# mumianyuxin/M3DSSD

Hardware: AMD Instinct MI355X
Metric: images/sec at 1280x384 bs=8, 1/2/4/8 MI355X; 3D-box Linf vs ref (higher is better)
Workload: dtype f32; 1 GPU; BASELINE.json configs[1]: full M3d_inference_align (DLA-34 + DCNv2 align + ANAB) forward + decode + top-3000 + NMS, bs=8/GPU, 1280x384, fp32, random-init synthetic weights and frames; per_gpu_batch=8, global_batch=8, parallelism=dp1 (batch sharded, 1 all-gather of [B,40,14] detections)

## Files before the change

### include/m3dssd_hip.h

```cpp
#ifndef M3DSSD_HIP_H
#define M3DSSD_HIP_H

#include <stdint.h>

#ifdef __cplusplus
extern "C" {
#endif

typedef void *m3d_stream_t;

enum {
    M3D_OK = 0,
    M3D_E_ARG = -1,
    M3D_E_HIP = -2,
    M3D_E_WORKSPACE = -3
};

const char *m3d_last_error(void);
#define M3D_ABI_VERSION 5
int m3d_abi_version(void);
const char *m3d_source_hashes(void);

typedef struct m3d_conv_desc {
    const float *in;
// ... 17 lines not shown
    int sigmoid_from;
    const float *dcn_offmask;
    int dcn_om_cs;
    float *splitk_ws;
    long long splitk_ws_bytes;
} m3d_conv_desc;

int m3d_conv2d_forward(const m3d_conv_desc *d, m3d_stream_t stream);
int m3d_conv2d_splitk_plan(const m3d_conv_desc *d, int *splits, long long *ws_bytes);

int m3d_conv_wave_applicable(const m3d_conv_desc *d);
int m3d_conv_wave_splitk_plan(const m3d_conv_desc *d, int *splits, long long *ws_bytes);
int m3d_conv_wave_forward(const m3d_conv_desc *d, m3d_stream_t stream);
int m3d_conv_wave_forward_wgsplit(const m3d_conv_desc *d, m3d_stream_t stream);
int m3d_conv_wave_wgsplit_width(const m3d_conv_desc *d, int *slices, int *width);

int m3d_wino_conv3x3_forward(const m3d_conv_desc *d, m3d_stream_t stream);
int m3d_wino_conv3x3_variant(const m3d_conv_desc *d);
int m3d_wino_conv3x3_splitk_plan(const m3d_conv_desc *d, int *splits, long long *ws_bytes);
int m3d_wino_conv3x3_forward_ex(const m3d_conv_desc *d, int variant, m3d_stream_t stream);
int m3d_wino44_applicable(const m3d_conv_desc *d);
int m3d_wino44_conv3x3_forward(const m3d_conv_desc *d, m3d_stream_t stream);
int m3d_wino44_conv3x3_forward_ex(const m3d_conv_desc *d, int nb, m3d_stream_t stream);
int m3d_wino44_kpair(const m3d_conv_desc *d);
int m3d_wino44_splitk_plan(const m3d_conv_desc *d, int *splits, long long *ws_bytes);
int m3d_wino44_conv3x3_forward_touch(const m3d_conv_desc *d, int nb, const void *touch, long long touch_bytes, m3d_stream_t stream);

int m3d_cache_touch(const void *p, long long bytes, m3d_stream_t stream);
int m3d_upload_indirect(const void *const *src_slot, void *dst, long long bytes, m3d_stream_t stream);

// ... 315 lines not shown
```

### m3dssd_amd/_hip.py

```python
import ctypes
import os
import subprocess

_HERE = os.path.dirname(os.path.abspath(__file__))
CSRC = os.path.join(_HERE, "csrc")
SO_PATH = os.environ.get("M3D_HIP_LIB") or os.path.join(CSRC, "build", "libm3dssd_hip.so")
HEADER = os.path.join(os.path.dirname(_HERE), "include", "m3dssd_hip.h")

c_int, c_float, c_ll, c_void_p = ctypes.c_int, ctypes.c_float, ctypes.c_longlong, ctypes.c_void_p


class ConvDesc(ctypes.Structure):
    _fields_ = [
        ("inp", c_void_p), ("in_cs", c_int),
        ("N", c_int), ("H", c_int), ("W", c_int), ("Cin", c_int),
        ("wgt", c_void_p), ("wgt_img_stride", c_ll),
        ("Cout", c_int), ("Cout_pad", c_int),
        ("kh", c_int), ("kw", c_int), ("stride", c_int), ("pad", c_int), ("dil", c_int),
        ("Ho", c_int), ("Wo", c_int),
        ("out", c_void_p), ("out_cs", c_int), ("out_nchw", c_int), ("out_img_stride", c_ll),
        ("scale", c_void_p), ("shift", c_void_p),
        ("res", c_void_p), ("res_cs", c_int), ("res_mode", c_int),
        ("act", c_int), ("sigmoid_from", c_int),
        ("dcn_offmask", c_void_p), ("dcn_om_cs", c_int),
# ... 113 lines not shown
    "m3d_wino_conv3x3_splitk_plan": (c_int, [ctypes.POINTER(ConvDesc), ctypes.POINTER(c_int), ctypes.POINTER(c_ll)]),
    "m3d_wino_conv3x3_variant": (c_int, [ctypes.POINTER(ConvDesc)]),
    "m3d_wino44_applicable": (c_int, [ctypes.POINTER(ConvDesc)]),
    "m3d_wino44_conv3x3_forward": (c_int, [ctypes.POINTER(ConvDesc), P]),
    "m3d_wino44_conv3x3_forward_ex": (c_int, [ctypes.POINTER(ConvDesc), c_int, P]),
    "m3d_wino44_kpair": (c_int, [ctypes.POINTER(ConvDesc)]),
    "m3d_wino44_conv3x3_forward_touch": (c_int, [ctypes.POINTER(ConvDesc), c_int, P, c_ll, P]),
    "m3d_cache_touch": (c_int, [P, c_ll, P]),
    "m3d_upload_indirect": (c_int, [P, P, c_ll, P]),
    "m3d_wino44_splitk_plan": (c_int, [ctypes.POINTER(ConvDesc), ctypes.POINTER(c_int), ctypes.POINTER(c_ll)]),
    "m3d_conv_wave_applicable": (c_int, [ctypes.POINTER(ConvDesc)]),
    "m3d_conv_wave_splitk_plan": (c_int, [ctypes.POINTER(ConvDesc), ctypes.POINTER(c_int), ctypes.POINTER(c_ll)]),
    "m3d_conv_wave_forward": (c_int, [ctypes.POINTER(ConvDesc), P]),
    "m3d_conv_wave_forward_wgsplit": (c_int, [ctypes.POINTER(ConvDesc), P]),
    "m3d_conv_wave_wgsplit_width": (c_int, [ctypes.POINTER(ConvDesc), ctypes.POINTER(c_int), ctypes.POINTER(c_int)]),
    "m3d_conv2d_tile": (c_int, [ctypes.POINTER(ConvDesc)] + [ctypes.POINTER(c_int)] * 4),
    "m3d_conv2d_splitk_plan": (c_int, [ctypes.POINTER(ConvDesc), ctypes.POINTER(c_int), ctypes.POINTER(c_ll)]),
    "m3d_dcn_v2_workspace_bytes": (c_ll, [c_int] * 10),
    "m3d_dcn_v2_workspace_bytes_grouped": (c_ll, [c_int] * 11),
    "m3d_dcn_v2_forward": (c_int, [P] * 6 + [c_int] * 14 + [P, c_ll, P]),
    "m3d_dcn_v2_backward_workspace_bytes": (c_ll, [c_int] * 11),
    "m3d_dcn_v2_backward": (c_int, [P] * 10 + [c_int] * 14 + [P, c_ll, P]),
    "m3d_rpn_loss_workspace_bytes": (c_ll, [c_int, c_ll]),
    "m3d_rpn_targets": (c_int, [P, c_int, c_int, c_int, P, c_int, P, c_int, c_int, P, P, c_int, P, P, P, P, P, c_ll, P]),
    "m3d_rpn_loss": (c_int, [P, c_int, c_int, c_int, P, c_int, P, c_int, c_int, P, P, P, c_int, P, P, P, P, P, P, P, P, P, P, c_ll, P]),
    "m3d_pack_conv_weight": (c_int, [P, P] + [c_int] * 6 + [P]),
    "m3d_nchw_to_nhwc": (c_int, [P, P] + [c_int] * 5 + [P]),
    "m3d_nhwc_to_nchw": (c_int, [P, c_int, P] + [c_int] * 4 + [P]),
    "m3d_stem_conv7x7": (c_int, [P, P, P, P, P] + [c_int] * 4 + [P]),
    "m3d_refine_3d": (c_int, [P, P, c_int, c_int, P, P, ctypes.c_double, c_int, ctypes.c_double, ctypes.c_double, P, P]),
# ... 92 lines not shown
```

### m3dssd_amd/csrc/dcn_wave.hip

```cpp
#include <stdlib.h>

#include <type_traits>

#include "common.h"

struct ConvWaveArgs {
    const float *in, *wfrag, *scale, *shift, *res, *om;
    float *out;
    int in_cs, out_cs, res_cs, om_cs;
    int H, W, Cin, Ho, Wo, HoWo, Cout;
    int kh, kw, stride, pad, dil;
    int M, KG, tiles_n;
    int act, res_mode, sigmoid_from;
    int vec_out;
    long long w_img_stride;
    unsigned in_bytes, out_bytes, res_bytes, w_bytes;
    float *ws;
    int splits, ss_per, base_waves;
    unsigned ws_bytes;
#ifdef CONV_TRACE
    long long *trace;
#endif
};


#ifdef CONV_TRACE
static long long *g_conv_trace = nullptr;
extern "C" void m3d_conv_wave_set_trace(void *buf) { g_conv_trace = (long long *)buf; }
static int g_conv_variant = 0;
extern "C" void m3d_conv_wave_set_variant(int v) { g_conv_variant = v; }
#define TRACE_INIT() long long *trp = (a.trace && threadIdx.x < 64) ? a.trace + (size_t)blockIdx.x * 128 : nullptr; int tri = 0
#define TRACE() do { if (trp && lane == 0 && tri < 128) trp[tri++] = __builtin_readcyclecounter(); } while (0)
#else
#define TRACE_INIT()
#define TRACE()
#endif

template <bool DEFORM, int NT, int NCQ = 4, int WPE = (DEFORM ? 2 : 3), int S = 1>
__global__ __launch_bounds__(64 * S) __attribute__((amdgpu_waves_per_eu(WPE))) void conv_wave_kernel(const ConvWaveArgs a)
{
    __shared__ __attribute__((aligned(16))) float tileS[S * 32 * 32];
    __shared__ __attribute__((aligned(16))) float tapst[(DEFORM ? 9 : 1) * 32 * 8];
    const int lane = threadIdx.x & 63, l31 = lane & 31, h = lane >> 5;
    const int wv = S > 1 ? __builtin_amdgcn_readfirstlane((int)threadIdx.x >> 6) : 0;
    float *const tileA = tileS + wv * 1024;
    const int gp = lane >> 3, gc = lane & 7;
    TRACE_INIT();
    TRACE();
    int blk;
    {
        const int nblk = gridDim.x, bid = blockIdx.x;
        const int q = nblk >> 3, r = nblk & 7, xcd = bid & 7, loc = bid >> 3;
        blk = (xcd < r ? xcd * (q + 1) : r * (q + 1) + (xcd - r) * q) + loc;
    }
    int split = wv;
    if (S == 1 && a.splits > 1) {
        split = blk / a.base_waves;
        blk -= split * a.base_waves;
    }
    const int bm = blk / a.tiles_n, bn = blk - bm * a.tiles_n;
    const int m0 = bm * 32;
    const int KK = a.kh * a.kw, C32 = a.Cin / 32;
    const bool idle = S > 1 && wv >= a.splits;
    const int ss0 = idle ? 0 : split * a.ss_per, ss1 = idle ? 0 : min(KK * C32, ss0 + a.ss_per);

    const __amdgpu_buffer_rsrc_t rin = make_rsrc(a.in, a.in_bytes);
// ... 111 lines not shown
    };

    f32x16 acc[NT];
#pragma unroll
    for (int nt = 0; nt < NT; ++nt)
#pragma unroll
        for (int r = 0; r < 16; ++r) acc[nt][r] = 0.f;

    int tap, c32;
    constexpr bool cmaj = DEFORM;
    if constexpr (cmaj) { c32 = ss0 / KK; tap = ss0 - c32 * KK; }
    else { tap = ss0 / C32; c32 = ss0 - tap * C32; }
    setup_tap(tap);
    issue_gather(c32);
    issue_b((tap * C32 + c32) * 4, bfA);

    unsigned wr_off[4], rd_off[4];
#pragma unroll
    for (int g = 0; g < 4; ++g) {
        const int r = 8 * g + gp;
        wr_off[g] = (unsigned)(r * 32 + ((gc ^ ((r >> 1) & 7)) * 4));
    }
#pragma unroll
    for (int j = 0; j < 4; ++j) rd_off[j] = (unsigned)(l31 * 32 + (((2 * j + h) ^ ((l31 >> 1) & 7)) * 4));

    TRACE();
    for (int st = ss0; st < ss1; ++st) {
        TRACE();
        const int kg0 = (tap * C32 + c32) * 4;
#pragma unroll
// ... 229 lines not shown
                const int m = mb + (r & 3) + 8 * (r >> 2);
                const unsigned ro = (cok && m < a.M) ? ((unsigned)m * (unsigned)a.res_cs + (unsigned)co) * 4u : M3D_BUF_OOB;
                rv[r] = __builtin_bit_cast(float, __builtin_amdgcn_raw_buffer_load_b32(rres, ro, 0, 0));
            }
        }
#pragma unroll
        for (int r = 0; r < 16; ++r) {
            const int m = mb + (r & 3) + 8 * (r >> 2);
            float v = conv_epi_affine(acc[nt][r], sc, sh, a.res ? rv[r] : 0.f, a.res != nullptr, a.res_mode);
            v = conv_epi_act(v, a.sigmoid_from >= 0 && co >= a.sigmoid_from, a.act == 1 ? M3D_LEAKY_SLOPE : 1.f);
            const unsigned oo = (cok && m < a.M) ? ((unsigned)m * (unsigned)a.out_cs + (unsigned)co) * 4u : M3D_BUF_OOB;
            __builtin_amdgcn_raw_buffer_store_b32(__builtin_bit_cast(unsigned, v), rout, oo, 0, 0);
        }
    }
    TRACE();
}

static int conv_wave_plan(const m3d_conv_desc *d, bool enforce_min, int *splits, int *ss_per, bool allow32 = false)
{
    *splits = 1;
    *ss_per = d->kh * d->kw * (d->Cin / 32);
    if (d->out_nchw) return 0;
    if (d->dcn_offmask && d->kh * d->kw > 9) return 0;
    if (d->Cin % 32 != 0 || d->Cout_pad % 32 != 0) return 0;
    if (d->Cout_pad % 64 != 0 && (!allow32 || d->dcn_offmask || d->wgt_img_stride)) return 0;
    const int cw = d->Cout_pad % 128 == 0 ? 128 : (d->Cout_pad % 64 == 0 ? 64 : 32);
    if (d->wgt_img_stride && (d->Ho * d->Wo) % 32 != 0) return 0;
    const long long M = (long long)d->N * d->Ho * d->Wo;
    const long long base = ((M + 31) / 32) * (d->Cout_pad / cw);
    if (base >= (1ll << 28)) return 0;
// ... 34 lines not shown
    *ws_bytes = (*splits > 1 && d->Cout_pad % 64 == 0) ? (long long)*splits * d->N * d->Ho * d->Wo * d->Cout_pad * 4 : 0;
    return M3D_OK;
}

template <bool DEFORM, int NT>
static void launch_wgsplit(const ConvWaveArgs &a, int S, int wgs, hipStream_t stream)
{
    constexpr int WPE = DEFORM ? 2 : 3;
    switch (S) {
    case 2: hipLaunchKernelGGL((conv_wave_kernel<DEFORM, NT, 4, WPE, 2>), dim3(wgs), dim3(128), 0, stream, a); break;
    case 4: hipLaunchKernelGGL((conv_wave_kernel<DEFORM, NT, 4, WPE, 4>), dim3(wgs), dim3(256), 0, stream, a); break;
    default: hipLaunchKernelGGL((conv_wave_kernel<DEFORM, NT, 4, WPE, 8>), dim3(wgs), dim3(512), 0, stream, a); break;
    }
}

static int conv_wave_run(const m3d_conv_desc *d_, hipStream_t stream, bool wgsplit)
{
    M3D_REQUIRE(d_ && d_->in && d_->wgt && d_->out, "conv_wave: null pointer");
    m3d_conv_desc dd = *d_;
    static float dummy;
    if (wgsplit) { dd.splitk_ws = &dummy; dd.splitk_ws_bytes = 0; }
    const m3d_conv_desc *d = &dd;
    int splits = 1, ss_per = 0;
    const int waves = conv_wave_plan(d, false, &splits, &ss_per, wgsplit);
    M3D_REQUIRE(waves > 0, "conv_wave: needs Cin %% 32 == 0, Cout_pad %% 64 == 0 (%% 32: plain, shared weights, wgsplit entry), NHWC output, "
                           "Ho*Wo %% 32 == 0 with per-image weights");
    const int ho = (d->H + 2 * d->pad - (d->dil * (d->kh - 1) + 1)) / d->stride + 1;
    const int wo = (d->W + 2 * d->pad - (d->dil * (d->kw - 1) + 1)) / d->stride + 1;
    M3D_REQUIRE(ho == d->Ho && wo == d->Wo, "conv_wave: Ho/Wo mismatch");
    M3D_REQUIRE(d->in_cs % 32 == 0 && d->in_cs >= d->Cin && ((uintptr_t)d->in & 127) == 0 && ((uintptr_t)d->wgt & 15) == 0,
                "conv_wave: the input view must be 128-byte aligned with in_cs %% 32 == 0");
    const long long M = (long long)d->N * d->Ho * d->Wo;
    M3D_REQUIRE(!d->wgt_img_stride || (d->wgt_img_stride % 4 == 0 && d->stride == 1 && d->Ho == d->H && d->Wo == d->W),
                "conv_wave: per-image weights need an image-aligned 16-byte stride and a same-size output");
    M3D_REQUIRE((long long)d->N * d->H * d->W * d->in_cs * 4 < (1ll << 31) && M * d->out_cs * 4 < (1ll << 31) &&
                M * d->res_cs * 4 < (1ll << 31) && (long long)d->Cout_pad * d->kh * d->kw * d->Cin * 4 < (1ll << 31),
                "conv_wave: views must be < 2 GiB");
    ConvWaveArgs a;
    a.in = d->in; a.wfrag = d->wgt; a.scale = d->scale; a.shift = d->shift; a.res = d->res; a.om = d->dcn_offmask;
    a.out = d->out;
    a.in_cs = d->in_cs; a.out_cs = d->out_cs; a.res_cs = d->res_cs; a.om_cs = d->dcn_om_cs;
    a.H = d->H; a.W = d->W; a.Cin = d->Cin; a.Ho = d->Ho; a.Wo = d->Wo; a.HoWo = d->Ho * d->Wo; a.Cout = d->Cout;
    a.kh = d->kh; a.kw = d->kw; a.stride = d->stride; a.pad = d->pad; a.dil = d->dil;
    const int cw = d->Cout_pad % 128 == 0 ? 128 : (d->Cout_pad % 64 == 0 ? 64 : 32);
    a.M = (int)M; a.KG = d->kh * d->kw * d->Cin / 8; a.tiles_n = d->Cout_pad / cw;
    a.act = d->act; a.res_mode = d->res_mode; a.sigmoid_from = d->sigmoid_from; a.w_img_stride = d->wgt_img_stride;
    static int vec_epi = -1;
    if (vec_epi < 0) { const char *e = getenv("M3D_WAVE_VEC_EPILOGUE"); vec_epi = e ? atoi(e) : 1; }
    a.vec_out = vec_epi && d->out_cs % 4 == 0 && ((uintptr_t)d->out & 15) == 0 &&
                (!d->res || (d->res_cs % 4 == 0 && ((uintptr_t)d->res & 15) == 0)) &&
                (!d->scale || ((uintptr_t)d->scale & 15) == 0) && (!d->shift || ((uintptr_t)d->shift & 15) == 0);
    a.in_bytes = (unsigned)((long long)d->N * d->H * d->W * d->in_cs * 4);
    a.out_bytes = (unsigned)(M * d->out_cs * 4);
    a.res_bytes = (unsigned)(M * d->res_cs * 4);
    a.w_bytes = (unsigned)((long long)cw * d->kh * d->kw * d->Cin * 4);
#ifdef CONV_TRACE
    a.trace = g_conv_trace;
#endif
    a.ws = nullptr; a.splits = 1; a.ss_per = ss_per; a.base_waves = waves; a.ws_bytes = 0;
    if (splits > 1 && wgsplit) {
        const int S = splits <= 2 ? 2 : (splits <= 4 ? 4 : 8);
        M3D_REQUIRE(splits <= 8, "conv_wave: %d K slices do not fit a workgroup", splits);
        a.splits = splits; a.base_waves = waves / splits;
        if (cw == 128) {
            if (d->dcn_offmask) launch_wgsplit<true, 4>(a, S, a.base_waves, stream);
            else launch_wgsplit<false, 4>(a, S, a.base_waves, stream);
        } else if (cw == 64) {
            if (d->dcn_offmask) launch_wgsplit<true, 2>(a, S, a.base_waves, stream);
            else launch_wgsplit<false, 2>(a, S, a.base_waves, stream);
        } else {
            launch_wgsplit<false, 1>(a, S, a.base_waves, stream);
        }
        M3D_LAUNCH_CHECK();
        return M3D_OK;
// ... 31 lines not shown
    if (splits > 1) {
        SplitkReduceArgs r;
        r.ws = a.ws; r.scale = d->scale; r.shift = d->shift; r.res = d->res; r.out = d->out;
        r.M = (int)M; r.Cout = d->Cout; r.Cout_pad = d->Cout_pad; r.splits = splits; r.out_cs = d->out_cs; r.res_cs = d->res_cs;
        r.res_mode = d->res_mode; r.act = d->act; r.sigmoid_from = d->sigmoid_from;
        return m3d_launch_splitk_reduce(r, stream);
    }
    return M3D_OK;
}

extern "C" int m3d_conv_wave_forward(const m3d_conv_desc *d, m3d_stream_t stream)
{
    return conv_wave_run(d, (hipStream_t)stream, false);
}

extern "C" int m3d_conv_wave_wgsplit_width(const m3d_conv_desc *d, int *slices, int *width)
{
    M3D_REQUIRE(d && slices && width, "conv_wave_wgsplit_width: null pointer");
    m3d_conv_desc t = *d;
    static float dummy;
    t.splitk_ws = &dummy;
    int p;
    const int waves = conv_wave_plan(&t, false, slices, &p, true);
    M3D_REQUIRE(waves > 0 && *slices <= 8, "conv_wave_wgsplit_width: the wave kernel does not apply to this descriptor");
    *width = *slices <= 1 ? 1 : (*slices <= 2 ? 2 : (*slices <= 4 ? 4 : 8));
    return M3D_OK;
}

extern "C" int m3d_conv_wave_forward_wgsplit(const m3d_conv_desc *d, m3d_stream_t stream)
{
// ... 3 lines not shown
```

### m3dssd_amd/engine.py

```python
import ctypes
import math
import os

import numpy as np
import torch

from . import _hip
from ._hip import ConvDesc, MlpDesc
from .config import model_flags

BN_EPS = 1e-5
SELECT_KEYS = os.environ.get("M3D_SELECT_KEYS", "1") != "0"
PSP_SIZES = (1, 4, 8, 16)
BACKBONE_CHANNELS = {"dla34": (16, 32, 64, 128, 256, 512), "dla102": (16, 32, 128, 256, 512, 1024)}
DLA102_LEVELS = (1, 1, 1, 3, 4, 1)


def _rup(a, b):
    return (a + b - 1) // b * b


class View:
    __slots__ = ("t", "ptr", "n", "h", "w", "c", "cs", "keep")

# ... 103 lines not shown
def pack_wino44_c16(weight, device):
    g = weight.detach().to("cpu", torch.float64)
    assert tuple(g.shape) == (16, 16, 3, 3)
    u = torch.einsum("ai,ocij,bj->abco", _WINO44_G, g, _WINO44_G).reshape(36, 4, 4, 16)
    return u.permute(0, 1, 3, 2).contiguous().to(torch.float32).reshape(-1).to(device)


WINO_MIN_BLOCKS = int(os.environ.get("M3D_WINO_MIN_BLOCKS", "128"))
FUSED_ANAB = os.environ.get("M3D_FUSED_ANAB", "1") != "0"
USE_ANAB_WAVE = os.environ.get("M3D_ANAB_WAVE", "1") != "0"
USE_ANAB_NESTED = os.environ.get("M3D_ANAB_NESTED", "1") != "0"
USE_DCN_WAVE = os.environ.get("M3D_DCN_WAVE", "1") != "0"
USE_CONV_WAVE = os.environ.get("M3D_CONV_WAVE", "1") != "0"
USE_CONV_WAVE_WGSPLIT = os.environ.get("M3D_CONV_WAVE_WGSPLIT", "1") != "0"
USE_OFFMASK_WAVE = os.environ.get("M3D_OFFMASK_WAVE", "1") != "0"
USE_WINO = os.environ.get("M3D_WINO", "1") != "0"
USE_WINO44 = os.environ.get("M3D_WINO44", "1") != "0"
WINO44_TOUCH = os.environ.get("M3D_WINO44_TOUCH", "1") != "0"
WINO44_TOUCH_SPAN = int(os.environ.get("M3D_WINO44_TOUCH_SPAN", "2"))
USE_WINO44_SPLITK = os.environ.get("M3D_WINO44_SPLITK", "1") != "0"
W44_SPLIT_NB = 2 if os.environ.get("M3D_W44_SPLIT_NB", "1") == "2" else 1
W44_SPLIT_KPAIR = os.environ.get("M3D_W44_SPLIT_NB", "1") == "3"
WINO44_MIN_WGS = int(os.environ.get("M3D_WINO44_MIN_WGS", "1000000"))
WINO44_MIN_WGS_NB1 = int(os.environ.get("M3D_WINO44_MIN_WGS_NB1", "200"))


class OpCost:

    def __init__(self, hbm_bytes):
        self.hbm_bytes = int(hbm_bytes)


def lo_hi_contains(start, end, n, br):
    lo, hi = start, (n if end is None else end)
    return lo <= br[0] and br[2] <= hi


class _Plan:

    def __init__(self):
        self.ops = []
        self.keep = []
        self.named = {}
        self.w44_prev = None
        self.branches = []


class Engine:
    def __init__(self, state_dict, conf, device=None, backbone_only=False):
        self.L = _hip.lib()
        self.backbone_only = backbone_only
        self.device = torch.device(device if device is not None else conf.device)
        if self.device.type != "cuda":
            raise NotImplementedError("the M3DSSD HIP engine runs on a ROCm device only (got %s)" % self.device)
        if self.device.index is None:
            self.device = torch.device("cuda", torch.cuda.current_device())
        self.conf = conf
        self.back_bone = str(conf.back_bone) if "back_bone" in conf else "dla34"
        if self.back_bone not in BACKBONE_CHANNELS:
            raise NotImplementedError("back_bone %r: the engine runs %s" % (self.back_bone, " / ".join(BACKBONE_CHANNELS)))
# ... 201 lines not shown
            if ssplits.value > 1:
                ws = torch.empty(sbytes.value // 4, device=self.device, dtype=torch.float32)
                plan.keep.append(ws)
                d.splitk_ws, d.splitk_ws_bytes = ws.data_ptr(), sbytes.value
                nb, ks44 = W44_SPLIT_NB, ssplits.value
        if w44ok and nb:
            u44 = pc.wino44()
            plan.keep.append(u44)
            d.wgt = u44.data_ptr()
            flops = 2.0 * x.n * d.Ho * d.Wo * d.Cout * 9 * pc.cin
            nxt = {"ptr": None, "bytes": 0}
            if WINO44_TOUCH:
                nbytes = u44.numel() * 4
                if plan.w44_prev is not None and len(plan.ops) - plan.w44_prev[0] <= WINO44_TOUCH_SPAN:
                    plan.w44_prev[1]["ptr"], plan.w44_prev[1]["bytes"] = u44.data_ptr(), nbytes
                else:
                    plan.ops.append((name + ".touch", "touch", 0.0,
                                     lambda st: _hip.check(L.m3d_cache_touch(u44.data_ptr(), nbytes, st)), OpCost(nbytes)))
            plan.w44_prev = (len(plan.ops), nxt)
            kp = ",kpair" if (nb == 1 and ((ks44 == 1 and L.m3d_wino44_kpair(ref) == 1) or (ks44 > 1 and W44_SPLIT_KPAIR))) else ""
            plan.ops.append((name, "wino44<16,%d%s%s>" % (16 * nb, ",splitk%d" % ks44 if ks44 > 1 else "", kp), flops,
                             lambda st: _hip.check(L.m3d_wino44_conv3x3_forward_touch(ref, nb, nxt["ptr"], nxt["bytes"], st)), d))
            return
        if (pc is not None and wgt_ptr is None and getattr(pc, "wino", None) is not None and kh == 3 and kw == 3
                and stride == 1 and pad == 1 and om is None and planar is None and x.h % 2 == 0 and x.w % 2 == 0
                and wino_blocks >= WINO_MIN_BLOCKS):
            d.wgt = pc.wino.data_ptr()
            flops = 2.0 * x.n * d.Ho * d.Wo * d.Cout * 9 * pc.cin
            ssplits, sbytes = ctypes.c_int(), ctypes.c_longlong()
            _hip.check(L.m3d_wino_conv3x3_splitk_plan(ref, ctypes.byref(ssplits), ctypes.byref(sbytes)))
# ... 11 lines not shown
            cin_true if cin_true is not None else (pc.cin if (pc is not None and wgt_ptr is None) else x.c))
        if wgt_frag:
            assert wgt_ptr is not None and planar is None and x.cs % 32 == 0 and x.ptr % 128 == 0, name
            if L.m3d_conv_wave_applicable(ref) <= 0:
                raise RuntimeError("%s: fragment-ordered weights but the wave kernel does not apply" % name)
            plan.ops.append((name, "conv_wave", flops_true, lambda st: _hip.check(L.m3d_conv_wave_forward(ref, st)), d))
            return
        if (pc is not None and wgt_ptr is None and planar is None and (USE_DCN_WAVE if om is not None else USE_CONV_WAVE)
                and x.cs % 32 == 0 and x.ptr % 128 == 0 and pc.cin_pad == x.c):
            wsplits, wbytes = ctypes.c_int(), ctypes.c_longlong()
            _hip.check(L.m3d_conv_wave_splitk_plan(ref, ctypes.byref(wsplits), ctypes.byref(wbytes)))
            if wsplits.value > 1 and USE_CONV_WAVE_WGSPLIT and (d.Cout_pad % 64 == 0 or (USE_OFFMASK_WAVE and wsplits.value <= 4)):
                frag = pc.frag()
                d.wgt = frag.data_ptr()
                kind = "conv_wave<%s>" % ",".join((["deform"] if om is not None else []) + ["wgsplit%d" % wsplits.value])
                plan.ops.append((name, kind, flops_true, lambda st: _hip.check(L.m3d_conv_wave_forward_wgsplit(ref, st)), d))
                return
            ws = None
            if wsplits.value > 1 and wbytes.value > 0:
                ws = torch.empty(wbytes.value // 4, device=self.device, dtype=torch.float32)
                d.splitk_ws, d.splitk_ws_bytes = ws.data_ptr(), wbytes.value
            if L.m3d_conv_wave_applicable(ref) > 0:
                frag = pc.frag()
                d.wgt = frag.data_ptr()
                if ws is not None:
                    plan.keep.append(ws)
                kind = "conv_wave%s" % ("<%s>" % ",".join(
                    (["deform"] if om is not None else []) + (["splitk%d" % wsplits.value] if wsplits.value > 1 else []))
                    if (om is not None or wsplits.value > 1) else "")
                plan.ops.append((name, kind, flops_true, lambda st: _hip.check(L.m3d_conv_wave_forward(ref, st)), d))
                return
            d.splitk_ws, d.splitk_ws_bytes = None, 0
        bm, bn, bk, grid = ctypes.c_int(), ctypes.c_int(), ctypes.c_int(), ctypes.c_int()
        _hip.check(L.m3d_conv2d_tile(ref, ctypes.byref(bm), ctypes.byref(bn), ctypes.byref(bk), ctypes.byref(grid)))
        splits, ws_bytes = ctypes.c_int(), ctypes.c_longlong()
        _hip.check(L.m3d_conv2d_splitk_plan(ref, ctypes.byref(splits), ctypes.byref(ws_bytes)))
        if splits.value > 1:
            ws = torch.empty(ws_bytes.value // 4, device=self.device, dtype=torch.float32)
            plan.keep.append(ws)
            d.splitk_ws, d.splitk_ws_bytes = ws.data_ptr(), ws_bytes.value
        kind = "igemm<%d,%d,%d%s%s%s>" % (bm.value, bn.value, bk.value, ",deform" if om is not None else "",
                                          ",planar" if planar is not None else "",
                                          ",splitk%d" % splits.value if splits.value > 1 else "")
        if cin_true is None:
            cin_true = pc.cin if (pc is not None and wgt_ptr is None) else x.c
        flops = 2.0 * x.n * d.Ho * d.Wo * d.Cout * kh * kw * cin_true
        plan.ops.append((name, kind, flops, lambda st: _hip.check(L.m3d_conv2d_forward(ref, st)), d))

    def _op(self, plan, name, kind, fn, flops=0.0, nbytes=None):
        plan.ops.append((name, kind, float(flops), fn, OpCost(nbytes) if nbytes is not None else None))

    def _build_plan(self, B, H, W):
        L, P = self.L, self.P
        plan = _Plan()
        chs = BACKBONE_CHANNELS[self.back_bone]
        b = "base.base"
        in_ptr = [0]
        plan.named["input_ptr"] = in_ptr
        s0 = self._buf(plan, B, H, W, 16)
        in_u8 = [0, 0, 0]
        plan.named["input_u8"] = in_u8
        mean3 = (ctypes.c_float * 3)(*[float(v) for v in self.conf.image_means])
# ... 23 lines not shown
            self._conv(plan, "level0", P["level0"], s0, l0, 1, 1, act=1)
        l1 = self._buf(plan, B, H // 2, W // 2, 32, name="level1")
        self._conv(plan, "level1", P["level1"], l0, l1, 2, 1, act=1)

        def maxpool(name, x, out):
            self._op(plan, name, "maxpool", lambda st: _hip.check(L.m3d_maxpool2x2(
                x.ptr, x.cs, out.ptr, out.cs, x.n, x.h, x.w, x.c, st)), nbytes=x.n * x.h * x.w * x.c * 5)

        if self.back_bone == "dla102":
            l3, l4, l5 = self._dla102_levels(plan, l1, maxpool)
        else:
            def block(p, x, res, out, stride):
                co = P[p + ".conv1"].cout
                t = self._buf(plan, B, out.h, out.w, co)
                self._conv(plan, p + ".conv1", P[p + ".conv1"], x, t, stride, 1, act=1)
                self._conv(plan, p + ".conv2", P[p + ".conv2"], t, out, 1, 1, act=1, res=res)

            def tree1(p, x, co, stride, out, bottom=None):
                h, w = x.h // stride, x.w // stride
                cat = self._buf(plan, B, h, w, 2 * co)
                x2v, x1v = cat.slice(0, co), cat.slice(co, co)
                if stride == 1:
                    bottom = x
                elif bottom is None:
                    bottom = self._buf(plan, B, h, w, x.c)
                    maxpool(p + ".downsample", x, bottom)
                if (p + ".project") in P:
                    res = self._buf(plan, B, h, w, co)
                    self._conv(plan, p + ".project", P[p + ".project"], bottom, res, 1, 0, act=0)
                else:
# ... 27 lines not shown
            cat5 = self._buf(plan, B, h5, w5, 1024 + 256)
            bottom5 = cat5.slice(1024, 256)
            maxpool(b + ".level5.downsample", l4, bottom5)
            res5 = self._buf(plan, B, h5, w5, 512)
            self._conv(plan, b + ".level5.project", P[b + ".level5.project"], bottom5, res5, 1, 0, act=0)
            block(b + ".level5.tree1", l4, res5, cat5.slice(512, 512), 2)
            block(b + ".level5.tree2", cat5.slice(512, 512), cat5.slice(512, 512), cat5.slice(0, 512), 1)
            self._conv(plan, b + ".level5.root", P[b + ".level5.root"], cat5, l5, 1, 0, act=1)

        def deform(p, x, out):
            om = self._buf(plan, B, x.h, x.w, 27, 28)
            self._conv(plan, p + ".offset_mask", P[p + ".om"], x, om, 1, 1, act=0, sigmoid_from=18)
            self._conv(plan, p + ".dcn", P[p + ".dcn"], x, out, 1, 1, act=1, om=om)
            plan.named[p + ".out"] = out

        def ida_step(p, i, x, skip, co):
            proj = self._buf(plan, B, x.h, x.w, co)
            deform("%s.proj_%d" % (p, i), x, proj)
            summed = self._buf(plan, B, 2 * x.h, 2 * x.w, co)
            upw = P["%s.up_%d" % (p, i)]
            self._op(plan, "%s.up_%d" % (p, i), "upsample", lambda st: _hip.check(L.m3d_upsample2x_add(
                proj.ptr, proj.cs, upw.data_ptr(), skip.ptr, skip.cs, summed.ptr, summed.cs, B, proj.h, proj.w, co, st)),
                flops=2.0 * B * 4 * proj.h * proj.w * co * 4, nbytes=B * proj.h * proj.w * co * 4 * (1 + 4 + 4))
            node = self._buf(plan, B, 2 * x.h, 2 * x.w, co)
            deform("%s.node_%d" % (p, i), summed, node)
            return node

        c3, c4 = chs[3], chs[4]
        L5a = ida_step("base.dla_up.ida_0", 1, l5, l4, c4)
        L4b = ida_step("base.dla_up.ida_1", 1, l4, l3, c3)
        L5b = ida_step("base.dla_up.ida_1", 2, L5a, L4b, c3)
        feats0 = ida_step("base.ida_up", 1, L5a, L5b, c3)
        plan.named["feats0"] = feats0

        plan.feat = (feats0.h, feats0.w)
        if self.backbone_only:
            return plan

        fh, fw = feats0.h, feats0.w
        HW = fh * fw
        A, NC = self.A, self.NC
        R = A * HW
        cls_pl = torch.empty(B * NC * A * HW, device=self.device, dtype=torch.float32)
        box_pl = torch.empty(B * 11 * A * HW, device=self.device, dtype=torch.float32)
        plan.keep += [cls_pl, box_pl]
        plan.named["cls_planar"], plan.named["box_planar"] = cls_pl, box_pl
        plan.named["planar_first_op"] = len(plan.ops)
# ... 57 lines not shown

        def box_ptr(k):
            return box_pl.data_ptr() + 4 * k * A * HW

        with_shape, with_center, with_anab = self.flags
        if with_shape:
            om_sa = self._buf(plan, B, fh, fw, 27, 28)
            self._op(plan, "shape_align.offsets", "align", lambda st: _hip.check(L.m3d_align_offsets(
                0, sel_idx.data_ptr(), sel_prob.data_ptr(), 0.5, P["shape.table"].data_ptr(), None, None, None, 0.0, 1.0, 0.0,
                1.0, om_sa.ptr, om_sa.cs, B, A, HW, 9, 0, st)), nbytes=B * HW * (2 + 28) * 4)
            feats = self._buf(plan, B, fh, fw, c3, name="feats")
            self._conv(plan, "shape_align.dcn", P["shape_align"], feats0, feats, 1, 1, act=0, res=feats0, om=om_sa)
        else:
            feats = plan.named["feats"] = feats0

        def center_align(p, x, kx, ky, mi, out):
            om = self._buf(plan, B, fh, fw, 3, 4)
            self._op(plan, p + ".offsets", "align", lambda st: _hip.check(L.m3d_align_offsets(
                1, sel_idx.data_ptr(), sel_prob.data_ptr(), 0.5, None, box_ptr(kx), box_ptr(ky),
                P["anchor_wh"].data_ptr(), float(means[mi]), float(stds[mi]), float(means[mi + 1]),
                float(stds[mi + 1]), om.ptr, om.cs, B, A, HW, 1, 11 * A * HW, st)), nbytes=B * HW * (2 + 2 + 4) * 4)
            self._conv(plan, p + ".dcn", P[p], x, out, 1, 0, act=0, res=x, om=om)

        z3d_now = [] if with_anab else ["bbox_z3d"]
        if with_center:
            heads([("bbox_x", feats, box_planar(0)), ("bbox_y", feats, box_planar(1)),
                   ("bbox_x3d", feats, box_planar(4)), ("bbox_y3d", feats, box_planar(5))])
            f2d = self._buf(plan, B, fh, fw, c3, name="feats_align2d")
            center_align("center_align2d", feats, 0, 1, 0, f2d)
            f3d = self._buf(plan, B, fh, fw, c3, name="feats_align3d")
            center_align("center_align3d", feats, 4, 5, 4, f3d)
            heads([("bbox_w", f2d, box_planar(2)), ("bbox_h", f2d, box_planar(3))] +
                  [(h, f3d, box_planar(self.box_heads.index(h))) for h in z3d_now + ["bbox_w3d", "bbox_h3d", "bbox_l3d", "bbox_rY3d"]])
        else:
            f2d = f3d = plan.named["feats_align2d"] = plan.named["feats_align3d"] = feats
            heads([(h, feats, box_planar(k)) for k, h in enumerate(self.box_heads) if h != "bbox_z3d" or not with_anab])

        if with_anab:
            gl = self._buf(plan, B, fh, fw, c3, name="feats_gl")
            self._anab_ops(plan, f3d, gl, P["anab.bn.scale"], P["anab.bn.shift"], act=1, res_mode=1)
            head("bbox_z3d", gl, box_planar(6))
        else:
            plan.named["feats_gl"] = f3d

        cls = torch.empty(B, R, NC, device=self.device, dtype=torch.float32)
        prob = torch.empty(B, R, NC, device=self.device, dtype=torch.float32)
# ... 223 lines not shown
        B, _, H, W = x.shape
        plan = self.plan_for(B, H, W)
        x = x.contiguous()
        plan.named["input_ptr"][0] = x.data_ptr()
        self.run_plan(plan)
        return plan.named["feats0"]

    def run_plan(self, plan, start=0, end=None):
        with torch.cuda.device(self.device):
            self._run_plan(plan, start, end)

    def _run_plan(self, plan, start, end):
        st = _Stream.current(self.device)
        ops = plan.ops[start:end]
        if self.profile is None:
            brs = [br for br in getattr(plan, "branches", ()) if lo_hi_contains(start, end, len(plan.ops), br)]
            if brs:
                lo, hi = start, (len(plan.ops) if end is None else end)
                main = torch.cuda.current_stream(self.device)
                if getattr(self, "_side", None) is None:
                    self._side = torch.cuda.Stream(self.device)
                side = self._side
                sst = ctypes.c_void_p(side.cuda_stream)
                forks = {br[0] for br in brs}
                joins = {br[2] for br in brs}
                on_side = set()
                for b0, b1, _ in brs:
                    on_side.update(range(b0, b1))
                for i in range(lo, hi):
                    if i in joins:
                        main.wait_stream(side)
                    if i in forks:
                        side.wait_stream(main)
                    plan.ops[i][3](sst if i in on_side else st)
                if hi in joins:
                    main.wait_stream(side)
                return
            for op in ops:
                op[3](st)
            return
        L = self.L
        evs = []
        for op in ops:
            if self.profile_kinds is not None and op[1] not in self.profile_kinds:
                op[3](st)
                continue
            e0, e1 = ctypes.c_void_p(), ctypes.c_void_p()
            _hip.check(L.m3d_event_create(ctypes.byref(e0)))
            _hip.check(L.m3d_event_create(ctypes.byref(e1)))
            _hip.check(L.m3d_event_record(e0, st))
            op[3](st)
            _hip.check(L.m3d_event_record(e1, st))
            evs.append((op, e0, e1))
        self._pending += evs
# ... 11 lines not shown
```

Baseline: 1402 images/sec.

## Batch independent wave-conv layers into one grouped launch with fused cache touch

Adds a batched conv_wave kernel that runs up to eight independent convolutions in one launch. Each workgroup maps to its layer through start offsets, and layers are sorted so the longest run first. The engine groups sibling layers: project/conv1 pairs, the three IDA offset-mask and DCN layers, and the two center-align DCNs. It also folds the Winograd weight cache-touch prefetch into the preceding wave launch. The intent is to cut launch count and tail under-occupancy for small layers, at the cost of shared launch bounds and extra rules on when layers may be grouped.

```diff
diff --git a/include/m3dssd_hip.h b/include/m3dssd_hip.h
--- a/include/m3dssd_hip.h
+++ b/include/m3dssd_hip.h
@@ -55,6 +55,7 @@
 int m3d_conv_wave_forward(const m3d_conv_desc *d, m3d_stream_t stream);
 int m3d_conv_wave_forward_wgsplit(const m3d_conv_desc *d, m3d_stream_t stream);
 int m3d_conv_wave_wgsplit_width(const m3d_conv_desc *d, int *slices, int *width);
+int m3d_conv_wave_forward_batched(const m3d_conv_desc *d, int n, const void *touch, long long touch_bytes, m3d_stream_t stream);
 
 int m3d_wino_conv3x3_forward(const m3d_conv_desc *d, m3d_stream_t stream);
 int m3d_wino_conv3x3_variant(const m3d_conv_desc *d);
diff --git a/m3dssd_amd/_hip.py b/m3dssd_amd/_hip.py
--- a/m3dssd_amd/_hip.py
+++ b/m3dssd_amd/_hip.py
@@ -151,6 +151,7 @@
     "m3d_conv_wave_forward": (c_int, [ctypes.POINTER(ConvDesc), P]),
     "m3d_conv_wave_forward_wgsplit": (c_int, [ctypes.POINTER(ConvDesc), P]),
     "m3d_conv_wave_wgsplit_width": (c_int, [ctypes.POINTER(ConvDesc), ctypes.POINTER(c_int), ctypes.POINTER(c_int)]),
+    "m3d_conv_wave_forward_batched": (c_int, [ctypes.POINTER(ConvDesc), c_int, P, c_ll, P]),
     "m3d_conv2d_tile": (c_int, [ctypes.POINTER(ConvDesc)] + [ctypes.POINTER(c_int)] * 4),
     "m3d_conv2d_splitk_plan": (c_int, [ctypes.POINTER(ConvDesc), ctypes.POINTER(c_int), ctypes.POINTER(c_ll)]),
     "m3d_dcn_v2_workspace_bytes": (c_ll, [c_int] * 10),
diff --git a/m3dssd_amd/csrc/dcn_wave.hip b/m3dssd_amd/csrc/dcn_wave.hip
--- a/m3dssd_amd/csrc/dcn_wave.hip
+++ b/m3dssd_amd/csrc/dcn_wave.hip
@@ -36,8 +36,9 @@
 #define TRACE()
 #endif
 
-template <bool DEFORM, int NT, int NCQ = 4, int WPE = (DEFORM ? 2 : 3), int S = 1>
-__global__ __launch_bounds__(64 * S) __attribute__((amdgpu_waves_per_eu(WPE))) void conv_wave_kernel(const ConvWaveArgs a)
+template <bool DEFORM, int NT, int NCQ, int WPE, int S, bool BATCH>
+__device__ __forceinline__ void conv_wave_body(const ConvWaveArgs a, const int bid, const int nblk, const char *touch,
+                                               const int touch_lines)
 {
     __shared__ __attribute__((aligned(16))) float tileS[S * 32 * 32];
     __shared__ __attribute__((aligned(16))) float tapst[(DEFORM ? 9 : 1) * 32 * 8];
@@ -47,9 +48,16 @@
     const int gp = lane >> 3, gc = lane & 7;
     TRACE_INIT();
     TRACE();
+    float touched = 0.f;
+    if constexpr (BATCH) {
+        if (touch) {
+            const int nthr = (int)gridDim.x * (64 * S);
+            for (int i = (int)blockIdx.x * (64 * S) + (int)threadIdx.x; i < touch_lines; i += nthr)
+                asm volatile("global_load_dword %0, %1, off" : "=v"(touched) : "v"(touch + (size_t)i * 128) : "memory");
+        }
+    }
     int blk;
     {
-        const int nblk = gridDim.x, bid = blockIdx.x;
         const int q = nblk >> 3, r = nblk & 7, xcd = bid & 7, loc = bid >> 3;
         blk = (xcd < r ? xcd * (q + 1) : r * (q + 1) + (xcd - r) * q) + loc;
     }
@@ -191,6 +199,7 @@
     setup_tap(tap);
     issue_gather(c32);
     issue_b((tap * C32 + c32) * 4, bfA);
+    if constexpr (BATCH) asm volatile("s_waitcnt vmcnt(0)" : "+v"(touched) : : "memory");
 
     unsigned wr_off[4], rd_off[4];
 #pragma unroll
@@ -450,6 +459,31 @@
         }
     }
     TRACE();
+}
+
+template <bool DEFORM, int NT, int NCQ = 4, int WPE = (DEFORM ? 2 : 3), int S = 1>
+__global__ __launch_bounds__(64 * S) __attribute__((amdgpu_waves_per_eu(WPE))) void conv_wave_kernel(const ConvWaveArgs a)
+{
+    conv_wave_body<DEFORM, NT, NCQ, WPE, S, false>(a, blockIdx.x, gridDim.x, nullptr, 0);
+}
+
+#define CONV_WAVE_BATCH_MAX 8
+struct ConvWaveBatch {
+    ConvWaveArgs op[CONV_WAVE_BATCH_MAX];
+    int start[CONV_WAVE_BATCH_MAX];
+    int nblk[CONV_WAVE_BATCH_MAX];
+    const char *touch;
+    int touch_lines;
+};
+
+template <bool DEFORM, int NT, int S>
+__global__ __launch_bounds__(64 * S) __attribute__((amdgpu_waves_per_eu(DEFORM ? 2 : 3))) void conv_wave_batched_kernel(const ConvWaveBatch b)
+{
+    const int gbid = blockIdx.x;
+    int op = 0;
+#pragma unroll
+    for (int i = 1; i < CONV_WAVE_BATCH_MAX; ++i) op += gbid >= b.start[i] ? 1 : 0;
+    conv_wave_body<DEFORM, NT, 4, (DEFORM ? 2 : 3), S, true>(b.op[op], gbid - b.start[op], b.nblk[op], b.touch, b.touch_lines);
 }
 
 static int conv_wave_plan(const m3d_conv_desc *d, bool enforce_min, int *splits, int *ss_per, bool allow32 = false)
@@ -514,15 +548,16 @@
     }
 }
 
-static int conv_wave_run(const m3d_conv_desc *d_, hipStream_t stream, bool wgsplit)
+static int conv_wave_fill(const m3d_conv_desc *d_, bool wgsplit, m3d_conv_desc &dd, ConvWaveArgs &a, int &waves, int &splits, int &cw)
 {
     M3D_REQUIRE(d_ && d_->in && d_->wgt && d_->out, "conv_wave: null pointer");
-    m3d_conv_desc dd = *d_;
+    dd = *d_;
     static float dummy;
     if (wgsplit) { dd.splitk_ws = &dummy; dd.splitk_ws_bytes = 0; }
     const m3d_conv_desc *d = &dd;
-    int splits = 1, ss_per = 0;
-    const int waves = conv_wave_plan(d, false, &splits, &ss_per, wgsplit);
+    int ss_per = 0;
+    splits = 1;
+    waves = conv_wave_plan(d, false, &splits, &ss_per, wgsplit);
     M3D_REQUIRE(waves > 0, "conv_wave: needs Cin %% 32 == 0, Cout_pad %% 64 == 0 (%% 32: plain, shared weights, wgsplit entry), NHWC output, "
                            "Ho*Wo %% 32 == 0 with per-image weights");
     const int ho = (d->H + 2 * d->pad - (d->dil * (d->kh - 1) + 1)) / d->stride + 1;
@@ -536,13 +571,12 @@
     M3D_REQUIRE((long long)d->N * d->H * d->W * d->in_cs * 4 < (1ll << 31) && M * d->out_cs * 4 < (1ll << 31) &&
                 M * d->res_cs * 4 < (1ll << 31) && (long long)d->Cout_pad * d->kh * d->kw * d->Cin * 4 < (1ll << 31),
                 "conv_wave: views must be < 2 GiB");
-    ConvWaveArgs a;
     a.in = d->in; a.wfrag = d->wgt; a.scale = d->scale; a.shift = d->shift; a.res = d->res; a.om = d->dcn_offmask;
     a.out = d->out;
     a.in_cs = d->in_cs; a.out_cs = d->out_cs; a.res_cs = d->res_cs; a.om_cs = d->dcn_om_cs;
     a.H = d->H; a.W = d->W; a.Cin = d->Cin; a.Ho = d->Ho; a.Wo = d->Wo; a.HoWo = d->Ho * d->Wo; a.Cout = d->Cout;
     a.kh = d->kh; a.kw = d->kw; a.stride = d->stride; a.pad = d->pad; a.dil = d->dil;
-    const int cw = d->Cout_pad % 128 == 0 ? 128 : (d->Cout_pad % 64 == 0 ? 64 : 32);
+    cw = d->Cout_pad % 128 == 0 ? 128 : (d->Cout_pad % 64 == 0 ? 64 : 32);
     a.M = (int)M; a.KG = d->kh * d->kw * d->Cin / 8; a.tiles_n = d->Cout_pad / cw;
     a.act = d->act; a.res_mode = d->res_mode; a.sigmoid_from = d->sigmoid_from; a.w_img_stride = d->wgt_img_stride;
     static int vec_epi = -1;
@@ -558,6 +592,18 @@
     a.trace = g_conv_trace;
 #endif
     a.ws = nullptr; a.splits = 1; a.ss_per = ss_per; a.base_waves = waves; a.ws_bytes = 0;
+    return M3D_OK;
+}
+
+static int conv_wave_run(const m3d_conv_desc *d_, hipStream_t stream, bool wgsplit)
+{
+    m3d_conv_desc dd;
+    ConvWaveArgs a;
+    int waves = 0, splits = 1, cw = 0;
+    const int rc = conv_wave_fill(d_, wgsplit, dd, a, waves, splits, cw);
+    if (rc != M3D_OK) return rc;
+    const m3d_conv_desc *d = &dd;
+    const long long M = (long long)d->N * d->Ho * d->Wo;
     if (splits > 1 && wgsplit) {
         const int S = splits <= 2 ? 2 : (splits <= 4 ? 4 : 8);
         M3D_REQUIRE(splits <= 8, "conv_wave: %d K slices do not fit a workgroup", splits);
@@ -619,6 +665,86 @@
     return conv_wave_run(d, (hipStream_t)stream, false);
 }
 
+template <bool DEFORM, int NT>
+static void launch_batched(const ConvWaveBatch &b, int S, int wgs, hipStream_t stream)
+{
+    switch (S) {
+    case 1: hipLaunchKernelGGL((conv_wave_batched_kernel<DEFORM, NT, 1>), dim3(wgs), dim3(64), 0, stream, b); break;
+    case 2: hipLaunchKernelGGL((conv_wave_batched_kernel<DEFORM, NT, 2>), dim3(wgs), dim3(128), 0, stream, b); break;
+    case 4: hipLaunchKernelGGL((conv_wave_batched_kernel<DEFORM, NT, 4>), dim3(wgs), dim3(256), 0, stream, b); break;
+    default: hipLaunchKernelGGL((conv_wave_batched_kernel<DEFORM, NT, 8>), dim3(wgs), dim3(512), 0, stream, b); break;
+    }
+}
+
+extern "C" int m3d_conv_wave_forward_batched(const m3d_conv_desc *d, int n, const void *touch, long long touch_bytes,
+                                             m3d_stream_t stream_)
+{
+    hipStream_t stream = (hipStream_t)stream_;
+    M3D_REQUIRE(d && n >= 1 && n <= CONV_WAVE_BATCH_MAX, "conv_wave_batched: 1..%d layers per launch (got %d)", CONV_WAVE_BATCH_MAX, n);
+    M3D_REQUIRE(touch_bytes >= 0 && touch_bytes / 128 < (1ll << 31) && (touch || touch_bytes == 0), "conv_wave_batched: touch range");
+    const bool touching = touch && touch_bytes >= 128;
+    if (n == 1 && !touching) return conv_wave_run(d, stream, true);
+    ConvWaveArgs args[CONV_WAVE_BATCH_MAX];
+    int wgs[CONV_WAVE_BATCH_MAX], order[CONV_WAVE_BATCH_MAX];
+    int S = 1, cw0 = 0;
+    long long total = 0;
+    for (int i = 0; i < n; ++i) {
+        m3d_conv_desc dd;
+        int waves = 0, splits = 1, cw = 0;
+        const int rc = conv_wave_fill(d + i, true, dd, args[i], waves, splits, cw);
+        if (rc != M3D_OK) return rc;
+        M3D_REQUIRE(!dd.wgt_img_stride, "conv_wave_batched: per-image weights are not taken (layer %d)", i);
+        M3D_REQUIRE(splits <= 8, "conv_wave: %d K slices do not fit a workgroup", splits);
+        if (i == 0) cw0 = cw;
+        M3D_REQUIRE(cw == cw0 && (d[i].dcn_offmask != nullptr) == (d[0].dcn_offmask != nullptr),
+                    "conv_wave_batched: the layers of one launch must share the channels per wave (128 / 64 / 32) and be all plain "
+                    "or all deformable (layer %d differs)", i);
+        args[i].splits = splits;
+        args[i].base_waves = wgs[i] = waves / splits;
+        const int w = splits <= 1 ? 1 : (splits <= 2 ? 2 : (splits <= 4 ? 4 : 8));
+        if (w > S) S = w;
+        total += wgs[i];
+        order[i] = i;
+    }
+    M3D_REQUIRE(total < (1ll << 28), "conv_wave_batched: too many workgroups");
+    static int longest_first = -1;
+    if (longest_first < 0) { const char *e = getenv("M3D_CONV_WAVE_BATCH_ORDER"); longest_first = e ? atoi(e) : 1; }
+    for (int i = 1; i < n; ++i)
+        for (int j = i; j > 0; --j) {
+            const int p = args[order[j - 1]].ss_per, q = args[order[j]].ss_per;
+            if (longest_first ? p >= q : p <= q) break;
+            const int t = order[j]; order[j] = order[j - 1]; order[j - 1] = t;
+        }
+    ConvWaveBatch b;
+    int at = 0;
+    for (int i = 0; i < CONV_WAVE_BATCH_MAX; ++i) {
+        if (i < n) {
+            b.op[i] = args[order[i]];
+            b.start[i] = at;
+            b.nblk[i] = wgs[order[i]];
+            at += wgs[order[i]];
+        } else {
+            b.op[i] = b.op[0];
+            b.start[i] = 0x7fffffff;
+            b.nblk[i] = 0;
+        }
+    }
+    b.touch = touching ? (const char *)touch : nullptr;
+    b.touch_lines = touching ? (int)(touch_bytes / 128) : 0;
+    const bool deform = d[0].dcn_offmask != nullptr;
+    if (cw0 == 128) {
+        if (deform) launch_batched<true, 4>(b, S, at, stream);
+        else launch_batched<false, 4>(b, S, at, stream);
+    } else if (cw0 == 64) {
+        if (deform) launch_batched<true, 2>(b, S, at, stream);
+        else launch_batched<false, 2>(b, S, at, stream);
+    } else {
+        launch_batched<false, 1>(b, S, at, stream);
+    }
+    M3D_LAUNCH_CHECK();
+    return M3D_OK;
+}
+
 extern "C" int m3d_conv_wave_wgsplit_width(const m3d_conv_desc *d, int *slices, int *width)
 {
     M3D_REQUIRE(d && slices && width, "conv_wave_wgsplit_width: null pointer");
diff --git a/m3dssd_amd/engine.py b/m3dssd_amd/engine.py
--- a/m3dssd_amd/engine.py
+++ b/m3dssd_amd/engine.py
@@ -141,6 +141,11 @@
 USE_CONV_WAVE = os.environ.get("M3D_CONV_WAVE", "1") != "0"
 USE_CONV_WAVE_WGSPLIT = os.environ.get("M3D_CONV_WAVE_WGSPLIT", "1") != "0"
 USE_OFFMASK_WAVE = os.environ.get("M3D_OFFMASK_WAVE", "1") != "0"
+WAVE_GROUP_TAGS = ("level2", "level3", "level4", "level5", "ida_om", "ida_dcn", "center", "touch")
+WAVE_GROUPS_DEFAULT = frozenset(WAVE_GROUP_TAGS) - {"level3"}
+_wg = os.environ.get("M3D_CONV_WAVE_GROUPS", "1")
+WAVE_GROUPS = frozenset() if _wg == "0" else (WAVE_GROUPS_DEFAULT if _wg == "1" else
+                                              frozenset(t for t in _wg.split(",") if t in WAVE_GROUP_TAGS))
 USE_WINO = os.environ.get("M3D_WINO", "1") != "0"
 USE_WINO44 = os.environ.get("M3D_WINO44", "1") != "0"
 WINO44_TOUCH = os.environ.get("M3D_WINO44_TOUCH", "1") != "0"
@@ -171,6 +176,8 @@
         self.named = {}
         self.w44_prev = None
         self.branches = []
+        self.groups = []
+        self.wave_ops = {}
 
 
 class Engine:
@@ -402,6 +409,9 @@
                 nbytes = u44.numel() * 4
                 if plan.w44_prev is not None and len(plan.ops) - plan.w44_prev[0] <= WINO44_TOUCH_SPAN:
                     plan.w44_prev[1]["ptr"], plan.w44_prev[1]["bytes"] = u44.data_ptr(), nbytes
+                elif "touch" in WAVE_GROUPS and (len(plan.ops) - 1) in plan.wave_ops:
+                    rec = plan.wave_ops[len(plan.ops) - 1][1]
+                    rec["ptr"], rec["bytes"] = u44.data_ptr(), nbytes
                 else:
                     plan.ops.append((name + ".touch", "touch", 0.0,
                                      lambda st: _hip.check(L.m3d_cache_touch(u44.data_ptr(), nbytes, st)), OpCost(nbytes)))
@@ -443,7 +453,7 @@
                 frag = pc.frag()
                 d.wgt = frag.data_ptr()
                 kind = "conv_wave<%s>" % ",".join((["deform"] if om is not None else []) + ["wgsplit%d" % wsplits.value])
-                plan.ops.append((name, kind, flops_true, lambda st: _hip.check(L.m3d_conv_wave_forward_wgsplit(ref, st)), d))
+                self._wave_op(plan, name, kind, flops_true, d, lambda st: _hip.check(L.m3d_conv_wave_forward_wgsplit(ref, st)))
                 return
             ws = None
             if wsplits.value > 1 and wbytes.value > 0:
@@ -457,7 +467,10 @@
                 kind = "conv_wave%s" % ("<%s>" % ",".join(
                     (["deform"] if om is not None else []) + (["splitk%d" % wsplits.value] if wsplits.value > 1 else []))
                     if (om is not None or wsplits.value > 1) else "")
-                plan.ops.append((name, kind, flops_true, lambda st: _hip.check(L.m3d_conv_wave_forward(ref, st)), d))
+                if ws is None:
+                    self._wave_op(plan, name, kind, flops_true, d, lambda st: _hip.check(L.m3d_conv_wave_forward(ref, st)))
+                else:
+                    plan.ops.append((name, kind, flops_true, lambda st: _hip.check(L.m3d_conv_wave_forward(ref, st)), d))
                 return
             d.splitk_ws, d.splitk_ws_bytes = None, 0
         bm, bn, bk, grid = ctypes.c_int(), ctypes.c_int(), ctypes.c_int(), ctypes.c_int()
@@ -475,6 +488,42 @@
             cin_true = pc.cin if (pc is not None and wgt_ptr is None) else x.c
         flops = 2.0 * x.n * d.Ho * d.Wo * d.Cout * kh * kw * cin_true
         plan.ops.append((name, kind, flops, lambda st: _hip.check(L.m3d_conv2d_forward(ref, st)), d))
+
+    def _wave_op(self, plan, name, kind, flops, d, fn):
+        if not WAVE_GROUPS:
+            plan.ops.append((name, kind, flops, fn, d))
+            return
+        L, ref, rec = self.L, ctypes.byref(d), {"ptr": None, "bytes": 0}
+
+        def run(st):
+            if rec["ptr"] is None:
+                fn(st)
+            else:
+                _hip.check(L.m3d_conv_wave_forward_batched(ref, 1, rec["ptr"], rec["bytes"], st))
+        plan.wave_ops[len(plan.ops)] = (d, rec)
+        plan.ops.append((name, kind, flops, run, d))
+
+    def _group(self, plan, tag, g0, g1):
+        idx = range(g0, g1)
+        if tag not in WAVE_GROUPS or g1 - g0 < 2 or not all(i in plan.wave_ops for i in idx):
+            return False
+        ds = [plan.wave_ops[i][0] for i in idx]
+        recs = [plan.wave_ops[i][1] for i in idx]
+        form = {(bool(d.dcn_offmask), 128 if d.Cout_pad % 128 == 0 else (64 if d.Cout_pad % 64 == 0 else 32)) for d in ds}
+        outs = {d.out for d in ds}
+        reads = {q for d in ds for q in (d.inp, d.res, d.dcn_offmask) if q}
+        if len(form) != 1 or len(outs) != len(ds) or outs & reads:
+            return False
+        L, n = self.L, len(ds)
+        arr = (ConvDesc * n)()
+        for i, d in enumerate(ds):
+            ctypes.memmove(ctypes.addressof(arr[i]), ctypes.addressof(d), ctypes.sizeof(ConvDesc))
+
+        def run(st):
+            t = next((r for r in recs if r["ptr"] is not None), recs[0])
+            _hip.check(L.m3d_conv_wave_forward_batched(arr, n, t["ptr"], t["bytes"], st))
+        plan.groups.append((g0, g1, run))
+        return True
 
     def _op(self, plan, name, kind, fn, flops=0.0, nbytes=None):
         plan.ops.append((name, kind, float(flops), fn, OpCost(nbytes) if nbytes is not None else None))
@@ -528,6 +577,9 @@
                 co = P[p + ".conv1"].cout
                 t = self._buf(plan, B, out.h, out.w, co)
                 self._conv(plan, p + ".conv1", P[p + ".conv1"], x, t, stride, 1, act=1)
+                i = len(plan.ops) - 1
+                if i >= 1 and plan.ops[i - 1][0].endswith(".project"):
+                    self._group(plan, p[len(b) + 1:].split(".")[0], i - 1, i + 1)
                 self._conv(plan, p + ".conv2", P[p + ".conv2"], t, out, 1, 1, act=1, res=res)
 
             def tree1(p, x, co, stride, out, bottom=None):
@@ -585,9 +637,10 @@
             self._conv(plan, p + ".dcn", P[p + ".dcn"], x, out, 1, 1, act=1, om=om)
             plan.named[p + ".out"] = out
 
-        def ida_step(p, i, x, skip, co):
-            proj = self._buf(plan, B, x.h, x.w, co)
-            deform("%s.proj_%d" % (p, i), x, proj)
+        def ida_step(p, i, x, skip, co, proj=None):
+            if proj is None:
+                proj = self._buf(plan, B, x.h, x.w, co)
+                deform("%s.proj_%d" % (p, i), x, proj)
             summed = self._buf(plan, B, 2 * x.h, 2 * x.w, co)
             upw = P["%s.up_%d" % (p, i)]
             self._op(plan, "%s.up_%d" % (p, i), "upsample", lambda st: _hip.check(L.m3d_upsample2x_add(
@@ -599,9 +652,23 @@
 
         c3, c4 = chs[3], chs[4]
         L5a = ida_step("base.dla_up.ida_0", 1, l5, l4, c4)
-        L4b = ida_step("base.dla_up.ida_1", 1, l4, l3, c3)
-        L5b = ida_step("base.dla_up.ida_1", 2, L5a, L4b, c3)
-        feats0 = ida_step("base.ida_up", 1, L5a, L5b, c3)
+        projs = [None] * 3
+        if WAVE_GROUPS & {"ida_om", "ida_dcn"}:
+            srcs = [("base.dla_up.ida_1.proj_1", l4), ("base.dla_up.ida_1.proj_2", L5a), ("base.ida_up.proj_1", L5a)]
+            projs = [self._buf(plan, B, x.h, x.w, c3) for _, x in srcs]
+            oms = [self._buf(plan, B, x.h, x.w, 27, 28) for _, x in srcs]
+            g0 = len(plan.ops)
+            for (p, x), om in zip(srcs, oms):
+                self._conv(plan, p + ".offset_mask", P[p + ".om"], x, om, 1, 1, act=0, sigmoid_from=18)
+            self._group(plan, "ida_om", g0, len(plan.ops))
+            g0 = len(plan.ops)
+            for (p, x), om, out in zip(srcs, oms, projs):
+                self._conv(plan, p + ".dcn", P[p + ".dcn"], x, out, 1, 1, act=1, om=om)
+                plan.named[p + ".out"] = out
+            self._group(plan, "ida_dcn", g0, len(plan.ops))
+        L4b = ida_step("base.dla_up.ida_1", 1, l4, l3, c3, projs[0])
+        L5b = ida_step("base.dla_up.ida_1", 2, L5a, L4b, c3, projs[1])
+        feats0 = ida_step("base.ida_up", 1, L5a, L5b, c3, projs[2])
         plan.named["feats0"] = feats0
 
         plan.feat = (feats0.h, feats0.w)
@@ -689,22 +756,33 @@
         else:
             feats = plan.named["feats"] = feats0
 
-        def center_align(p, x, kx, ky, mi, out):
-            om = self._buf(plan, B, fh, fw, 3, 4)
-            self._op(plan, p + ".offsets", "align", lambda st: _hip.check(L.m3d_align_offsets(
+        def center_align(p, x, kx, ky, mi, out, om=None, phase=3):
+            if phase & 1:
+                om = self._buf(plan, B, fh, fw, 3, 4)
+                self._op(plan, p + ".offsets", "align", lambda st: _hip.check(L.m3d_align_offsets(
                 1, sel_idx.data_ptr(), sel_prob.data_ptr(), 0.5, None, box_ptr(kx), box_ptr(ky),
-                P["anchor_wh"].data_ptr(), float(means[mi]), float(stds[mi]), float(means[mi + 1]),
-                float(stds[mi + 1]), om.ptr, om.cs, B, A, HW, 1, 11 * A * HW, st)), nbytes=B * HW * (2 + 2 + 4) * 4)
-            self._conv(plan, p + ".dcn", P[p], x, out, 1, 0, act=0, res=x, om=om)
+                    P["anchor_wh"].data_ptr(), float(means[mi]), float(stds[mi]), float(means[mi + 1]),
+                    float(stds[mi + 1]), om.ptr, om.cs, B, A, HW, 1, 11 * A * HW, st)), nbytes=B * HW * (2 + 2 + 4) * 4)
+            if phase & 2:
+                self._conv(plan, p + ".dcn", P[p], x, out, 1, 0, act=0, res=x, om=om)
+            return om
 
         z3d_now = [] if with_anab else ["bbox_z3d"]
         if with_center:
             heads([("bbox_x", feats, box_planar(0)), ("bbox_y", feats, box_planar(1)),
                    ("bbox_x3d", feats, box_planar(4)), ("bbox_y3d", feats, box_planar(5))])
             f2d = self._buf(plan, B, fh, fw, c3, name="feats_align2d")
-            center_align("center_align2d", feats, 0, 1, 0, f2d)
             f3d = self._buf(plan, B, fh, fw, c3, name="feats_align3d")
-            center_align("center_align3d", feats, 4, 5, 4, f3d)
+            if "center" in WAVE_GROUPS:
+                om2 = center_align("center_align2d", feats, 0, 1, 0, f2d, phase=1)
+                om3 = center_align("center_align3d", feats, 4, 5, 4, f3d, phase=1)
+                g0 = len(plan.ops)
+                center_align("center_align2d", feats, 0, 1, 0, f2d, om2, phase=2)
+                center_align("center_align3d", feats, 4, 5, 4, f3d, om3, phase=2)
+                self._group(plan, "center", g0, len(plan.ops))
+            else:
+                center_align("center_align2d", feats, 0, 1, 0, f2d)
+                center_align("center_align3d", feats, 4, 5, 4, f3d)
             heads([("bbox_w", f2d, box_planar(2)), ("bbox_h", f2d, box_planar(3))] +
                   [(h, f3d, box_planar(self.box_heads.index(h))) for h in z3d_now + ["bbox_w3d", "bbox_h3d", "bbox_l3d", "bbox_rY3d"]])
         else:
@@ -958,9 +1036,14 @@
         st = _Stream.current(self.device)
         ops = plan.ops[start:end]
         if self.profile is None:
+            lo, hi = start or 0, (len(plan.ops) if end is None else end)
+            if lo < 0 or hi < 0:
+                lo, hi, _ = slice(start, end).indices(len(plan.ops))
+            groups = {g0: (g1, fn) for g0, g1, fn in getattr(plan, "groups", ()) if lo <= g0 and g1 <= hi}
             brs = [br for br in getattr(plan, "branches", ()) if lo_hi_contains(start, end, len(plan.ops), br)]
+            forks, joins, on_side = set(), set(), set()
+            main = side = sst = None
             if brs:
-                lo, hi = start, (len(plan.ops) if end is None else end)
                 main = torch.cuda.current_stream(self.device)
                 if getattr(self, "_side", None) is None:
                     self._side = torch.cuda.Stream(self.device)
@@ -968,20 +1051,26 @@
                 sst = ctypes.c_void_p(side.cuda_stream)
                 forks = {br[0] for br in brs}
                 joins = {br[2] for br in brs}
-                on_side = set()
                 for b0, b1, _ in brs:
                     on_side.update(range(b0, b1))
-                for i in range(lo, hi):
-                    if i in joins:
-                        main.wait_stream(side)
-                    if i in forks:
-                        side.wait_stream(main)
-                    plan.ops[i][3](sst if i in on_side else st)
-                if hi in joins:
+                groups = {g0: g for g0, g in groups.items() if not any(
+                    j in forks or j in joins or (j in on_side) != (g0 in on_side) for j in range(g0 + 1, g[0]))}
+            i = lo
+            while i < hi:
+                if i in joins:
                     main.wait_stream(side)
-                return
-            for op in ops:
-                op[3](st)
+                if i in forks:
+                    side.wait_stream(main)
+                s_i = sst if i in on_side else st
+                if i in groups:
+                    g1, fn = groups[i]
+                    fn(s_i)
+                    i = g1
+                else:
+                    plan.ops[i][3](s_i)
+                    i += 1
+            if hi in joins:
+                main.wait_stream(side)
             return
         L = self.L
         evs = []
```

Result: no change. 1412 images/sec (median of 6 runs) (+0.7%).
